# hridaybavle/semantic_slam

Hardware: AMD Instinct MI355X
Metric: graph-optimize LM iters/sec (5k poses, 1k landmarks) (higher is better)
Workload: dtype f64

## Files before the change

semantic_slam_amd/csrc/chol_plan.hpp:

```cpp
#pragma once
#include <algorithm>
#include <array>
#include <cstdint>
#include <cstdio>
#include <cstdlib>
#include <cstring>
#include <functional>
#include <map>
#include <queue>
#include <string>
#include <unordered_map>
#include <utility>
#include <vector>

namespace sslam {
#ifdef SSLAM_PLAN_TIMERS
#include <chrono>
#define SSLAM_PT_INIT auto pt_ = std::chrono::steady_clock::now();
#define SSLAM_PT(name) { auto n_ = std::chrono::steady_clock::now(); fprintf(stderr, "[plan-timer] %-14s %.3f ms\n", name, std::chrono::duration<double, std::milli>(n_ - pt_).count()); pt_ = n_; }
#else
#define SSLAM_PT_INIT
#define SSLAM_PT(name)
#endif

struct ColMeta { int xoff, yoff, dim, graph, b0, nb, nbi, base, f0, f1, piece, ilevel; };

struct BlkMeta { int off, src, xoff_row, yoff_row, coldiag, colyoff, info, as0; };
constexpr int kBlkFmt = 1 << 8, kBlkDiag = 1 << 9, kBlkRowIn = 1 << 10, kBlkNasShift = 16;
inline int blk_irank_bits(int r) { return ((r & 31) << 11) | ((r >> 5) << 24); }
#if defined(__HIPCC__)
__host__ __device__
#endif
inline int blk_irank(int info) { return ((info >> 11) & 31) | (((info >> 24) & 255) << 5); }

struct AsmSrc { int uoff, uyoff; };
struct FwdMeta { int off, yoff; };

struct UpdMeta { unsigned ab, xk; };
constexpr unsigned kUpdDi6 = 1u << 28;
constexpr unsigned kUpdDk6 = 1u << 29;
constexpr unsigned kUpdDiag = 1u << 30;
constexpr unsigned kUpdDj6 = 1u << 31;
constexpr int kUpdLocalMax = 1 << 16, kUpdYMax = 1 << 13, kUpdRightYMax = 1 << 12;
#if defined(__HIPCC__)
#define SSLAM_HD_INLINE __host__ __device__ inline
#else
#define SSLAM_HD_INLINE inline
#endif
SSLAM_HD_INLINE int upd_ua(const UpdMeta& r) { return (int)(r.ab & 0xFFFFu); }
SSLAM_HD_INLINE int upd_ub(const UpdMeta& r) { return (int)(r.ab >> 16); }
SSLAM_HD_INLINE int upd_yk(const UpdMeta& r) { return (int)(r.xk & 0x1FFFu); }
SSLAM_HD_INLINE int upd_rt(const UpdMeta& r) { return (int)(r.xk & 0xFFFFu); }
SSLAM_HD_INLINE int upd_ry(const UpdMeta& r) { return (int)((r.xk >> 16) & 0xFFFu); }
inline UpdMeta upd_make(int ua_local, int ub_local, int yk_local, unsigned flags) { return UpdMeta{(unsigned)ua_local | ((unsigned)ub_local << 16), (unsigned)yk_local | flags}; }
inline UpdMeta upd_make_right(int ua_local, int ub_local, int tl, int yl, unsigned flags) { return UpdMeta{(unsigned)ua_local | ((unsigned)ub_local << 16), (unsigned)tl | ((unsigned)yl << 16) | flags}; }

}
#include "front_plan.hpp"
namespace sslam {

struct ItemMeta { int u0, n, tloff, flags; };
constexpr int kItemSole = 1;
constexpr int kItemSlotShift = 1, kItemSlotMask = 0x7FF, kItemYShift = 12;
struct MbMeta { int tloff, ps0, n, info; };
struct RCol { int u0, n; };
struct ILevel { int c0, c1, b0, b1, it0, it1, mb0, mb1; };

struct UItem { int u0, n, uoff, flags, s0, ns, uyoff, pad; };
constexpr int kUItemDi6 = 1 << 12, kUItemDj6 = 1 << 13, kUItemDiag = 1 << 14;
struct UMb { int uoff, ps0, n, info, s0, ns, uyoff, pad; };

struct PieceMeta { int graph, c0, nc, b0, nb, lbase, lsize, y0, ysize, ilv0, nilv, iit0, nit_i, iu0, nu_i, imb0, nimb, as0, nas, uit0, nuit, umb0, numb,
                   uu0, nuu, us0, nus, n36, n18, nint, pad3, pad4, nu4, nu2, nu1, pad5; };

inline int blk_doubles(int di, int dj) { return (di * dj + 1) & ~1; }
constexpr int kItemDoubles = 42;
constexpr int kMaxILevels = 64;

struct SymGraph { int prow0, nprow, lrow0, nlrow; int pp0 = 0, pp1 = 0, pl0 = 0, pl1 = 0, ll0 = 0, ll1 = 0; };
struct SymIn {
  int B = 0, nPr = 0, nLr = 0;
  std::vector<SymGraph> seg;
  std::vector<std::pair<int, int>> ppoff, plblk;
  std::vector<std::pair<int, int>> llblk;
  int64_t hll_base = 0, hpp_off_base = 0, hpl_base = 0, hll_off_base = 0;
};
// ... 34 lines not shown
        for (const char* v : legacy)
          if (getenv(v)) fprintf(stderr, "[sslam] %s is no longer read: plan options go through SSLAM_CHOL_OPTS=\"key=value,...\" (chol_plan.hpp CholOpts)\n", v);
      }
    }
    const char* e = getenv("SSLAM_CHOL_OPTS");
    if (!e) return;
    std::string str(e);
    size_t pos = 0;
    while (pos < str.size()) {
      size_t end = str.find(',', pos);
      if (end == std::string::npos) end = str.size();
      const std::string kv = str.substr(pos, end - pos);
      pos = end + 1;
      const size_t eq = kv.find('=');
      if (eq == std::string::npos) continue;
      const std::string k = kv.substr(0, eq), v = kv.substr(eq + 1);
      const int iv = atoi(v.c_str());
      if (k == "cap_leaf") cap_leaf = iv; else if (k == "cap_mid") cap_mid = iv; else if (k == "cap_tail") cap_tail = iv;
      else if (k == "max_blocks") max_blocks = iv; else if (k == "tail_width") tail_width = iv; else if (k == "mid_width") mid_width = iv;
      else if (k == "nt_leaf") { nt_leaf = iv; nt_leaf_set = true; } else if (k == "nt_mid") nt_mid = iv; else if (k == "nt_ftail") nt_ftail = iv; else if (k == "nt_bleaf") nt_bleaf = iv; else if (k == "nt_bmid") nt_bmid = iv; else if (k == "nt_btail") nt_btail = iv; else if (k == "nt_tail") nt_tail = iv;
      else if (k == "min_chunk") min_chunk = std::max(1, iv); else if (k == "split_min") split_min = std::max(2, iv);
      else if (k == "pcap_leaf") pcap_leaf = iv; else if (k == "pcap_mid") pcap_mid = iv; else if (k == "pcap_tail") pcap_tail = iv;
      else if (k == "group_cap") group_cap = iv; else if (k == "group_blocks") group_blocks = iv; else if (k == "ustage") ustage = iv;
      else if (k == "order_bits_max") order_bits_max = iv; else if (k == "flow") flow = iv; else if (k == "front") front = iv; else if (k == "compact") compact = iv; else if (k == "dump") dump = iv != 0;
      else if (k == "order") order = (v == "mindeg" || v == "0") ? 0 : 1;
      else if (k == "order_mul") order_mul = atof(v.c_str()); else if (k == "order_add") order_add = iv;
      else fprintf(stderr, "[sslam] SSLAM_CHOL_OPTS: unknown key '%s'\n", k.c_str());
    }
  }
  bool nt_leaf_set = false;
};

inline bool chol_throughput_regime(int B, int block_rows) { return B >= 32 || (B >= 2 && block_rows >= 8000); }
inline bool chol_opts_normalise(CholOpts& opt, int B, int block_rows) {
  auto one_of = [](int v, std::initializer_list<int> set) { return std::find(set.begin(), set.end(), v) != set.end(); };
  if (opt.nt_tail != 1024) opt.nt_tail = 512;
  if (!one_of(opt.nt_leaf, {-1, 128, 256, 512, 1024})) opt.nt_leaf = 64;
  if (!one_of(opt.nt_mid, {256, 512})) opt.nt_mid = 128;
  if (opt.nt_tail == 1024) opt.nt_ftail = 1024;
  else if (!one_of(opt.nt_ftail, {128, 256, 1024})) opt.nt_ftail = 512;
  if (!one_of(opt.nt_btail, {128, 256})) opt.nt_btail = 512;
  for (int* nt : {&opt.nt_bleaf, &opt.nt_bmid})
    if (*nt <= 0) *nt = 0;
    else if (!one_of(*nt, {128, 256, 512, 1024})) *nt = 64;
  const bool want_flow = opt.flow != 0 && B < 8 && !chol_throughput_regime(B, block_rows) && opt.nt_tail == 512 && opt.group_cap <= 0 && !opt.nt_leaf_set;
  if (want_flow) { opt.nt_leaf = opt.nt_tail; opt.mid_width = 0; }
  return want_flow;
}

struct CholHost {
  int ncol = 0, nlevels = 0, dim = 0, B = 0, npiece = 0;
  int64_t lnz = 0;
  int64_t unz = 0;
  std::vector<ColMeta> col; std::vector<BlkMeta> blk; std::vector<UpdMeta> upd; std::vector<ItemMeta> item; std::vector<MbMeta> mb;
  std::vector<ILevel> ilv; std::vector<PieceMeta> piece;
  std::vector<AsmSrc> asrc, usrc; std::vector<FwdMeta> fwd; std::vector<UItem> uitem; std::vector<UMb> umb;
  std::vector<RCol> rcol; std::vector<UpdMeta> rupd;
  std::vector<int> lvl_ptr, lvl_cols;
  std::vector<int> plv_ptr, plv_pieces;
  std::vector<PieceMeta> lpiece;
  std::vector<int> tail_ptr, tail_pieces;
  std::vector<int> plv_lds_f, plv_lds_b;
  std::vector<int> plv_nt, plv_cls;
  int tail_lds_f = 0, tail_lds_b = 0;
  int nt_leaf = 64, nt_mid = 128, nt_tail = 512, nt_ftail = 256, nt_bleaf = 0, nt_bmid = 0, nt_btail = 0, ustage = 0;
  bool front = false;
  std::string front_why;
  std::vector<uint32_t> fblob;
  std::vector<FrontGrp> fgrp, lfgrp;
  std::vector<int> plv_lds_ff;
  int tail_lds_ff = 0;
  int64_t funz = 0;
  std::string error;
};

namespace chol_detail {

struct GraphSym {
  std::vector<int> order;
  std::vector<int> cs_start, cs_len, cs_idx;
};

inline void min_degree(int n, std::vector<std::vector<int>>& adj, GraphSym& out) {
  std::vector<char> done(n, 0);
  using Item = std::pair<int, int>;
  std::priority_queue<Item, std::vector<Item>, std::greater<Item>> pq;
  for (int v = 0; v < n; ++v) { std::sort(adj[v].begin(), adj[v].end()); pq.push({(int)adj[v].size(), v}); }
  out.order.clear(); out.order.reserve(n);
  out.cs_start.assign(n, 0); out.cs_len.assign(n, 0); out.cs_idx.clear();
  std::vector<int> merged;
  while (!pq.empty()) {
    const Item it = pq.top(); pq.pop();
    const int v = it.second;
    if (done[v] || it.first != (int)adj[v].size()) continue;
    done[v] = 1;
    out.order.push_back(v);
    std::vector<int>& nb = adj[v];
    out.cs_start[v] = (int)out.cs_idx.size(); out.cs_len[v] = (int)nb.size(); out.cs_idx.insert(out.cs_idx.end(), nb.begin(), nb.end());
    for (int u : nb) {
      std::vector<int>& au = adj[u];
      merged.clear();
      merged.reserve(au.size() + nb.size());
      std::set_union(au.begin(), au.end(), nb.begin(), nb.end(), std::back_inserter(merged));
      au.clear();
      for (int w : merged) if (w != u && w != v) au.push_back(w);
      pq.push({(int)au.size(), u});
    }
// ... 436 lines not shown
    }
  }
  std::vector<int> plev(npiece, 0);
  for (int j = 0; j < ncol; ++j)
    if (bp[j + 1] - bp[j] > 1) {
      const int pp = col_piece[brow[bp[j] + 1]], pj = col_piece[j];
      if (pp != pj) plev[pp] = std::max(plev[pp], plev[pj] + 1);
    }
  int nplv = 0;
  for (int p = 0; p < npiece; ++p) if (!piece_tail[p]) nplv = std::max(nplv, plev[p] + 1);
  out.plv_ptr.assign(nplv + 1, 0);
  for (int p = 0; p < npiece; ++p) if (!piece_tail[p]) out.plv_ptr[plev[p] + 1]++;
  for (int l = 0; l < nplv; ++l) out.plv_ptr[l + 1] += out.plv_ptr[l];
  out.plv_pieces.resize(out.plv_ptr[nplv]);
  {
    std::vector<int> cursor(out.plv_ptr.begin(), out.plv_ptr.end() - 1);
    for (int p = 0; p < npiece; ++p) if (!piece_tail[p]) out.plv_pieces[cursor[plev[p]]++] = p;
  }
  out.tail_ptr.assign(B + 1, 0);
  for (int p = 0; p < npiece; ++p) if (piece_tail[p]) out.tail_ptr[out.piece[p].graph + 1]++;
  for (int g = 0; g < B; ++g) out.tail_ptr[g + 1] += out.tail_ptr[g];
  out.tail_pieces.resize(out.tail_ptr[B]);
  {
    std::vector<int> cursor(out.tail_ptr.begin(), out.tail_ptr.end() - 1);
    for (int p = 0; p < npiece; ++p) if (piece_tail[p]) out.tail_pieces[cursor[out.piece[p].graph]++] = p;
  }
  out.col.assign(ncol, ColMeta{});
  out.blk.assign(nblk, BlkMeta{});
  std::vector<int> block_col(nblk), col_nbi(ncol, 0);
  {
    std::vector<int> rowcnt(ncol + 1, 0);
    for (int j = 0; j < ncol; ++j) for (int t = bp[j] + 1; t < bp[j + 1]; ++t) rowcnt[brow[t] + 1]++;
    for (int j = 0; j < ncol; ++j) rowcnt[j + 1] += rowcnt[j];
    out.fwd.resize(rowcnt[ncol]);
    std::vector<int> cursor(rowcnt.begin(), rowcnt.end() - 1);
    for (int j = 0; j < ncol; ++j) {
      const int pj = col_piece[j];
      int nbi = 0;
      for (int t = bp[j]; t < bp[j + 1]; ++t) if (col_piece[brow[t]] == pj) ++nbi;
      for (int t = bp[j]; t < bp[j] + nbi; ++t) if (col_piece[brow[t]] != pj) { out.error = "in-piece rows of a column are not a prefix"; return -1; }
      col_nbi[j] = nbi;
      out.col[j] = ColMeta{col_xoff[j], col_yoff[j], col_dim[j], col_graph[j], bp[j], bp[j + 1] - bp[j], nbi, boff[bp[j]], rowcnt[j], rowcnt[j + 1], pj, col_il[j]};
      for (int t = bp[j]; t < bp[j + 1]; ++t) {
        const int i = brow[t];
        block_col[t] = j;
        BlkMeta& bm = out.blk[t];
        bm.off = boff[t]; bm.src = bsrc[t];
        bm.xoff_row = col_xoff[i]; bm.yoff_row = col_yoff[i]; bm.coldiag = boff[bp[j]]; bm.colyoff = col_yoff[j]; bm.as0 = 0;
        bm.info = col_dim[i] | (col_dim[j] << 4) | (bfmt[t] ? kBlkFmt : 0) | (t == bp[j] ? kBlkDiag : 0) | (col_piece[i] == pj ? kBlkRowIn : 0);
        if (t > bp[j]) out.fwd[cursor[i]++] = FwdMeta{boff[t] | (col_dim[j] == 6 ? (int)0x80000000u : 0), col_yoff[j]};
      }
    }
  }
  for (int p = 0; p < npiece; ++p) {
    PieceMeta& pm = out.piece[p];
    int r = 0;
    for (int t = pm.b0; t < pm.b0 + pm.nb; ++t)
      if (out.blk[t].info & kBlkRowIn) {
        if (r >= 8192) { out.error = "piece with more than 8191 row-in-piece blocks"; return -1; }
        out.blk[t].info |= blk_irank_bits(r++);
      }
    pm.nint = r;
  }
  SSLAM_PT("levels+cols")
  struct URec { int a, b, uoff, uy, comp; };
  std::vector<std::vector<URec>> inbox(npiece);
  std::vector<std::vector<int>> comp_R(ncomp);
  out.upd.clear(); out.item.clear(); out.mb.clear(); out.ilv.clear(); out.asrc.clear(); out.usrc.clear(); out.uitem.clear(); out.umb.clear();
  out.rupd.clear(); out.rcol.assign(ncol, RCol{0, 0});
  bool right_ok = true;
  std::vector<int> piece_pmax(npiece, 0);
  int64_t ucur = 0;
  struct UB { int comp, a, b; };
  struct OwnRec { int blk, ua, ubo, k; };
  struct SrcRec { int blk; AsmSrc s; };
  struct IU { int t, ua, ub2, k; };
  struct AsmRec { int t; AsmSrc s; };
  std::vector<UB> ub;
  std::vector<int> comps, ctab_base, ctab, rix, iu_ptr, as_ptr, own_ptr, src_ptr, cur1, cur2, cur3, cur4, bi0, bi1, order, uoffs;
  std::vector<OwnRec> own_flat, own_s;
  std::vector<SrcRec> src_flat;
  std::vector<IU> iu_flat, iu_s;
  std::vector<AsmRec> asm_flat;
  std::vector<AsmSrc> as_s, src_s;
  std::vector<int> lens, comp_uy;
  std::vector<UItem> uit_s;
  auto fit_chunk = [&](int lo, int hi, int pcap) {
    auto nonsole = [&](int chunk) { int s2 = 0; for (int n : lens) { const int k = (n + chunk - 1) / chunk; if (k > 1) s2 += k; } return s2; };
    if (lo >= hi || nonsole(lo) <= pcap) return lo;
    int a = lo, b = hi;
    while (b - a > 1) { const int m = a + (b - a) / 2; if (nonsole(m) <= pcap) b = m; else a = m; }
    return b;
  };
  for (int p = 0; p < npiece; ++p) {
    PieceMeta& pm = out.piece[p];
    const int nt = piece_tail[p] ? opt.nt_tail : (piece_cls[p] == 1 ? opt.nt_mid : opt.nt_leaf);
    const int slots = nt / 4;
    const int pcap = piece_tail[p] ? opt.pcap_tail : (piece_cls[p] == 1 ? opt.pcap_mid : opt.pcap_leaf);
    comps.clear();
    for (int j = pm.c0; j < pm.c0 + pm.nc; ++j) {
      if (comps.empty() || std::find(comps.begin(), comps.end(), col_comp[j]) == comps.end()) comps.push_back(col_comp[j]);
      std::vector<int>& R = comp_R[col_comp[j]];
      for (int t = bp[j] + col_nbi[j]; t < bp[j + 1]; ++t) R.push_back(brow[t]);
    }
    std::sort(comps.begin(), comps.end());
    for (int c : comps) {
      std::vector<int>& R = comp_R[c];
      std::sort(R.begin(), R.end());
      R.erase(std::unique(R.begin(), R.end()), R.end());
    }
    ub.clear();
    ctab_base.assign(comps.size() + 1, 0);
    for (size_t ci = 0; ci < comps.size(); ++ci) { const int r = (int)comp_R[comps[ci]].size(); ctab_base[ci + 1] = ctab_base[ci] + r * (r + 1) / 2; }
    ctab.assign(ctab_base.back(), -1);
    auto ublock = [&](int comp, int a, int b2) -> int {
// ... 180 lines not shown
        if (diag) {
          const std::vector<int>& R = comp_R[x.comp];
          uy = comp_uy[std::lower_bound(comps.begin(), comps.end(), x.comp) - comps.begin()] + 6 * (int)(std::lower_bound(R.begin(), R.end(), x.a) - R.begin());
        }
        const unsigned tpk = (di == 6 ? kUpdDi6 : 0u) | (diag ? kUpdDiag : 0u) | (dj == 6 ? kUpdDj6 : 0u);
        const int u0 = (int)out.upd.size() - pm.uu0;
        for (int w = own_ptr[q]; w < own_ptr[q + 1]; ++w) { const OwnRec& u = own_s[w]; out.upd.push_back(upd_make(u.ua - pm.lbase, u.ubo - pm.lbase, col_yoff[u.k] - pm.y0, tpk | (col_dim[u.k] == 6 ? kUpdDk6 : 0u))); }
        const int n = own_ptr[q + 1] - own_ptr[q];
        const int s0 = (int)out.usrc.size() - pm.us0;
        for (int w = src_ptr[q]; w < src_ptr[q + 1]; ++w) out.usrc.push_back(src_s[w]);
        const int ns = src_ptr[q + 1] - src_ptr[q];
        const int k = std::max(1, (n + chunk - 1) / chunk);
        const int shape = (di == 6 ? kUItemDi6 : 0) | (dj == 6 ? kUItemDj6 : 0) | (diag ? kUItemDiag : 0);
        for (int qq = 0; qq < k; ++qq) {
          const int a2 = u0 + qq * chunk, b2 = std::min(u0 + n, a2 + chunk);
          out.uitem.push_back(UItem{a2, std::max(0, b2 - a2), uoffs[q], shape | (k == 1 ? kItemSole : ((ps + qq) << kItemSlotShift)), s0, ns, uy, 0});
        }
        if (k > 1) { out.umb.push_back(UMb{uoffs[q], ps, k, di | (dj << 4) | (diag ? kBlkDiag : 0), s0, ns, uy, 0}); ps += k; }
        if (comp_dest[x.comp] < 0) { out.error = "a root component has an update matrix"; return -1; }
        inbox[comp_dest[x.comp]].push_back(URec{x.a, x.b, uoffs[q], uy, x.comp});
      }
      piece_pmax[p] = std::max(piece_pmax[p], ps);
      ucur = cur;
      {
        auto cls = [](const UItem& im) {
          if (!(im.flags & kItemSole)) return 3;
          const int t = ((im.flags & kUItemDi6) ? 2 : 1) * ((im.flags & kUItemDj6) ? 2 : 1);
          return t == 4 ? 0 : (t == 2 ? 1 : 2);
        };
        int cnt[4] = {0, 0, 0, 0};
        for (size_t i = item_first; i < out.uitem.size(); ++i) cnt[cls(out.uitem[i])]++;
        pm.nu4 = cnt[0]; pm.nu2 = cnt[1]; pm.nu1 = cnt[2];
        int at[4] = {0, cnt[0], cnt[0] + cnt[1], cnt[0] + cnt[1] + cnt[2]};
        uit_s.assign(out.uitem.begin() + item_first, out.uitem.end());
        for (const UItem& im : uit_s) out.uitem[item_first + at[cls(im)]++] = im;
      }
    }
    pm.nuit = (int)out.uitem.size() - pm.uit0;
    pm.numb = (int)out.umb.size() - pm.umb0;
    pm.nuu = (int)out.upd.size() - pm.uu0;
    pm.nus = (int)out.usrc.size() - pm.us0;
  }
  out.unz = ucur;
  SSLAM_PT("piece loop")
  if (!right_ok) { out.rupd.clear(); out.rcol.assign(ncol, RCol{0, 0}); }
  auto lds_f = [&](int p) {
    const PieceMeta& pm = out.piece[p];
    const int ustage = (piece_cls[p] >= 1 || !opt.ustage) ? 0 : 4 * pm.nuit + 4 * pm.numb + ((pm.nuu + 1) & ~1) + pm.nus + 2;
    return 4 * pm.nilv + ((pm.lsize + 1) & ~1) + 2 * ((pm.ysize + 1) & ~1) + 4 * pm.nb + 3 * pm.nc + 2 * pm.nit_i + ((pm.nu_i + 1) & ~1) + 2 * pm.nimb + pm.nas + ustage +
           kItemDoubles * piece_pmax[p] + 8 + (piece_cls[p] >= 1 ? pm.nc + 2 : 0);
  };
  auto lds_b = [&](int p) {
    const PieceMeta& pm = out.piece[p];
    return 4 * pm.nilv + 36 * pm.nint + ((pm.ysize + 1) & ~1) + 7 * pm.nb + 3 * pm.nc + 12;
  };
  {
    std::vector<int> ptr{0}, launch_order, lnt, lcls;
    launch_order.reserve(out.plv_pieces.size());
    const int cut[3] = {640, 853, 1280};
    for (int l = 0; l < nplv; ++l) {
      std::vector<int> ps, pmid;
      for (int q = out.plv_ptr[l]; q < out.plv_ptr[l + 1]; ++q) (piece_cls[out.plv_pieces[q]] == 1 ? pmid : ps).push_back(out.plv_pieces[q]);
      const int n = (int)ps.size();
      if (n >= opt.split_min) {
        std::stable_sort(ps.begin(), ps.end(), [&](int a, int b) { return lds_b(a) < lds_b(b); });
        int q0 = 0;
        for (int k = 0; k < 3 && q0 < n; ++k) {
          int q1 = q0;
          while (q1 < n && lds_b(ps[q1]) <= cut[k]) ++q1;
          if (q1 - q0 >= opt.split_min / 2 && n - q1 >= opt.split_min / 2) { for (int q = q0; q < q1; ++q) launch_order.push_back(ps[q]); ptr.push_back((int)launch_order.size()); lnt.push_back(opt.nt_leaf); lcls.push_back(0); q0 = q1; }
        }
        for (int q = q0; q < n; ++q) launch_order.push_back(ps[q]);
      } else {
        for (int p : ps) launch_order.push_back(p);
      }
      if ((int)launch_order.size() > ptr.back()) { ptr.push_back((int)launch_order.size()); lnt.push_back(opt.nt_leaf); lcls.push_back(0); }
      if (!pmid.empty()) { for (int p : pmid) launch_order.push_back(p); ptr.push_back((int)launch_order.size()); lnt.push_back(opt.nt_mid); lcls.push_back(1); }
    }
    out.plv_nt = lnt; out.plv_cls = lcls;
    out.plv_pieces = launch_order;
    out.plv_ptr = ptr;
  }
  const int nlaunch = (int)out.plv_ptr.size() - 1;
  out.lpiece.clear();
  out.lpiece.reserve(npiece);
  for (int p : out.plv_pieces) out.lpiece.push_back(out.piece[p]);
  for (int p : out.tail_pieces) out.lpiece.push_back(out.piece[p]);
  out.plv_lds_f.assign(nlaunch, 0); out.plv_lds_b.assign(nlaunch, 0);
  for (int l = 0; l < nlaunch; ++l)
    for (int q = out.plv_ptr[l]; q < out.plv_ptr[l + 1]; ++q) {
      out.plv_lds_f[l] = std::max(out.plv_lds_f[l], lds_f(out.plv_pieces[q]));
      out.plv_lds_b[l] = std::max(out.plv_lds_b[l], lds_b(out.plv_pieces[q]));
    }
  for (int p : out.tail_pieces) { out.tail_lds_f = std::max(out.tail_lds_f, lds_f(p)); out.tail_lds_b = std::max(out.tail_lds_b, lds_b(p)); }
  if (opt.front > 0) {
    FrontHost F;
    front_build(FrontIn{ncol, npiece, ncomp, bp, brow, boff, bsrc, bfmt, col_comp, col_piece, col_dim, col_xoff, col_yoff, col_il, comp_parent, comp_R}, out.piece, out.ilv, F);
    for (int p = 0; p < npiece && F.ok; ++p) {
      const int nt = piece_tail[p] ? opt.nt_ftail : (piece_cls[p] == 1 ? opt.nt_mid : opt.nt_leaf);
      for (int l = 0; l < out.piece[p].nilv; ++l) {
        const ILevel& lv = out.ilv[out.piece[p].ilv0 + l];
        if (lv.c1 - lv.c0 > 2 * (nt / 8)) { F.ok = false; F.why = "a level of a piece has more columns than the workgroup's teams hold"; break; }
      }
    }
    out.front = F.ok; out.front_why = F.why;
    if (F.ok) {
      out.fblob.swap(F.blob); out.fgrp.swap(F.grp); out.funz = F.unz;
      out.lfgrp.reserve(npiece);
      for (int p : out.plv_pieces) out.lfgrp.push_back(out.fgrp[p]);
      for (int p : out.tail_pieces) out.lfgrp.push_back(out.fgrp[p]);
      out.plv_lds_ff.assign(nlaunch, 0);
      for (int l = 0; l < nlaunch; ++l)
// ... 22 lines not shown
```

semantic_slam_amd/csrc/sslam_chol.hip:

```cpp
#include <hip/hip_runtime.h>
#include <algorithm>
#include <cstdio>
#include <cstring>
#include <mutex>
#include <type_traits>
#include <vector>

#include "../../include/sslam.h"
#include "graph_engine.hpp"
#include "chol_plan.hpp"

namespace sslam {

struct CholView {
  int ncol, nlevels, dim, npiece;
  const ColMeta* col;
  const BlkMeta* blk;
  const UpdMeta* upd;
  const ItemMeta* item;
  const MbMeta* mb;
  const ILevel* ilv;
  const PieceMeta* piece;
  const PieceMeta* lpiece;
  int ltail0;
  const AsmSrc* asrc;
  const AsmSrc* usrc;
  const UItem* uitem;
  const UMb* umb;
  const RCol* rcol;
  const UpdMeta* rupd;
  const int* plv_pieces;
  const int* tail_ptr;
  const int* tail_pieces;
  double* Lval;
  double* Uval;
  double* y;
  int* fail;
  const unsigned* fblob;
  const FrontGrp* lfgrp;
  int flat_L;
  long long* dbg;
};

struct SpecLanes {
  int K = 0;
  LmState* lm = nullptr;
  double *Lval = nullptr, *Uval = nullptr, *y = nullptr, *x = nullptr, *pose_trial = nullptr, *lmk_trial = nullptr, *part_e = nullptr, *part_a = nullptr;
  int *fail = nullptr, *flow = nullptr;
  int* err = nullptr;
  const double *pose_cur = nullptr, *lmk_cur = nullptr;
  long long sL = 0, sU = 0, sy = 0, sx = 0, spose = 0, slmk = 0, spe = 0, spa = 0, sflow = 0;
  int g0 = 0, g1 = 0;
  int after = 0;
  int* ctl = nullptr;
};

struct CholPlan {
  CholView C{};
  SpecLanes spec{};
  std::vector<int> plv_ptr, plv_lds_f, plv_lds_b, plv_nt, plv_cls;
  std::vector<int> plv_lds_ff;
  int tail_lds_ff = 0;
  bool front = false;
  int tail_lds_f = 0, tail_lds_b = 0, tail_total = 0, nt_tail = 512, nt_ftail = 256, nt_bleaf = 0, nt_bmid = 0, nt_btail = 0, ustage = 0;
  std::vector<void*> allocs;
  DevArena* arena = nullptr;
  int64_t lnz = 0, unz = 0;
  std::vector<int> lp_graph;
  std::vector<int> c_ptr;
  int* d_idx = nullptr;
// ... 658 lines not shown
  SSLAM_STAMP(6)
  if (C.flat_L) {
    D2* dst = reinterpret_cast<D2*>(C.Lval + pm.lbase);
    const D2* src = reinterpret_cast<const D2*>(smL);
    for (int e = tid; e < (pm.lsize >> 1); e += NT) dst[e] = src[e];
  } else {
    double* dst = C.Lval + pm.lbase;
    const int nA = pm.n36, nB = pm.n18, nC = pm.nb - nA - nB, eA = 36 * nA, eB = eA + 18 * nB;
    const float rA = 1.0f / (float)max(nA, 1), rB = 1.0f / (float)max(nB, 1), rC = 1.0f / (float)max(nC, 1);
    for (int t = tid; t < eA; t += NT) { const int k = (int)(((float)t + 0.5f) * rA), i = t - k * nA; dst[t] = smL[i * 36 + k]; }
    for (int t = tid; t < 18 * nB; t += NT) { const int k = (int)(((float)t + 0.5f) * rB), i = t - k * nB; dst[eA + t] = smL[eA + i * 18 + k]; }
    for (int t = tid; t < 9 * nC; t += NT) { const int k = (int)(((float)t + 0.5f) * rC), i = t - k * nC; dst[eB + t] = smL[eB + i * 10 + k]; }
  }
  for (int e = tid; e < pm.ysize; e += NT) C.y[pm.y0 + e] = smY[e];
  SSLAM_STAMP(7)
  if (dbg && threadIdx.x == 0) { dbg[8] += 1; dbg[9] += pm.nilv; dbg[10] += pm.nuit; dbg[11] += pm.nit_i; }
}
#undef SSLAM_STAMP

template <int NT, bool USTAGE, bool RIGHT = false>
__global__ __launch_bounds__(NT, 4) void k_chol_pieces(BatchView V, CholView C, int begin, const int* __restrict__ idx) {
  extern __shared__ double sm[];
  const PieceMeta pm = C.lpiece[idx ? idx[blockIdx.x] : begin + blockIdx.x];
  if (!V.lm[pm.graph].in_trial) return;
  chol_piece<NT, USTAGE, RIGHT>(V, C, pm, sm, (C.dbg && blockIdx.x == 0) ? C.dbg + 16 : nullptr);
}

template <int NT>
__global__ __launch_bounds__(NT) void k_chol_tail(BatchView V, CholView C, const int* __restrict__ idx) {
  extern __shared__ double sm[];
  const int g = idx ? idx[blockIdx.x] : blockIdx.x;
  if (!V.lm[g].in_trial) return;
  const int q1 = C.tail_ptr[g + 1];
  for (int q = C.tail_ptr[g]; q < q1; ++q) {
    if (C.rupd) chol_piece<NT, false, true>(V, C, C.lpiece[C.ltail0 + q], sm, (C.dbg && g == 0) ? C.dbg : nullptr);
    else chol_piece<NT, false, false>(V, C, C.lpiece[C.ltail0 + q], sm, (C.dbg && g == 0) ? C.dbg : nullptr);
    __threadfence_block();
    __syncthreads();
  }
}

#define SSLAM_BSTAMP(k)                                                         \
  if (dbg) {                                                                    \
    const long long now_ = clock64();                                           \
    if (threadIdx.x == 0) dbg[k] += now_ - tprev;                               \
    tprev = now_;                                                               \
  }
template <int NT>
__device__ __forceinline__ void chol_piece_backward(const CholView& C, const PieceMeta pm, const double* __restrict__ y, double* x, double* sm, long long* dbg) {
  ILevel* s_lvb = reinterpret_cast<ILevel*>(sm);
  long long tprev = dbg ? clock64() : 0;
  const int tid = threadIdx.x;
  const int Yp = (pm.ysize + 1) & ~1;
  double* smI = sm + 4 * pm.nilv;
  double* smX = smI + 36 * pm.nint;
  double* smE = smX + Yp;
  int2* sBlk = reinterpret_cast<int2*>(smE + 6 * pm.nb);
  int4* sCol = reinterpret_cast<int4*>(sBlk + pm.nb + (pm.nb & 1));
  int* sXoff = reinterpret_cast<int*>(sCol + pm.nc);
  const int nA = pm.n36, nB = pm.n18, nC = pm.nb - nA - nB, eA = 36 * nA, eB = eA + 18 * nB;
  const double y_r = y[pm.y0 + min(tid, pm.ysize - 1)];
  const ILevel lv_r = C.ilv[pm.ilv0 + min(tid, max(pm.nilv - 1, 0))];
  const ColMeta col_r = C.col[pm.c0 + min(tid, pm.nc - 1)];
  for (int b = tid; b < pm.nb; b += NT) {
    const BlkMeta bm = C.blk[pm.b0 + b];
    const int di = bm.info & 15, dj = (bm.info >> 4) & 15;
    const bool in = bm.info & kBlkRowIn;
    const int ol = bm.off - pm.lbase;
    int st, n, i;
    if (ol < eA) { st = 0; n = nA; i = ol / 36; }
    else if (ol < eB) { st = eA; n = nB; i = (ol - eA) / 18; }
    else { st = eB; n = nC; i = (ol - eB) / 10; }
    const double* __restrict__ g = C.Lval + pm.lbase + st + i;
    if (in) {
      const int lo = 36 * blk_irank(bm.info);
      sBlk[b] = make_int2(lo | (di << 24) | (dj << 28), bm.yoff_row - pm.y0);
      double* o = smI + lo;
      if (dj == 6) {
        for (int r = 0; r < di; r += 3) {
          double v[18];
#pragma unroll
          for (int k = 0; k < 18; ++k) v[k] = g[(size_t)(r * 6 + k) * n];
#pragma unroll
          for (int k = 0; k < 18; ++k) o[r * 6 + k] = v[k];
        }
      } else {
        for (int r = 0; r < di; r += 3) {
          double v[9];
#pragma unroll
          for (int k = 0; k < 9; ++k) v[k] = g[(size_t)(r * 3 + k) * n];
#pragma unroll
          for (int k = 0; k < 9; ++k) o[r * 3 + k] = v[k];
        }
      }
    } else {
      const double* xi = x + bm.xoff_row;
      double sv[6] = {0, 0, 0, 0, 0, 0};
      if (dj == 6) {
        for (int r = 0; r < di; r += 3) {
          double v[18];
          const double x0 = xi[r], x1 = xi[r + 1], x2 = xi[r + 2];
#pragma unroll
          for (int k = 0; k < 18; ++k) v[k] = g[(size_t)(r * 6 + k) * n];
#pragma unroll
          for (int c = 0; c < 6; ++c) { sv[c] += v[c] * x0; sv[c] += v[6 + c] * x1; sv[c] += v[12 + c] * x2; }
        }
      } else {
        for (int r = 0; r < di; r += 3) {
          double v[9];
          const double x0 = xi[r], x1 = xi[r + 1], x2 = xi[r + 2];
#pragma unroll
          for (int k = 0; k < 9; ++k) v[k] = g[(size_t)(r * 3 + k) * n];
#pragma unroll
          for (int c = 0; c < 3; ++c) { sv[c] += v[c] * x0; sv[c] += v[3 + c] * x1; sv[c] += v[6 + c] * x2; }
        }
      }
#pragma unroll
      for (int c = 0; c < 6; ++c) smE[b * 6 + c] = sv[c];
    }
  }
  if (tid < pm.ysize) smX[tid] = y_r;
  for (int e = tid + NT; e < pm.ysize; e += NT) smX[e] = y[pm.y0 + e];
  if (tid < pm.nilv) s_lvb[tid] = lv_r;
  for (int i = tid + NT; i < pm.nilv; i += NT) s_lvb[i] = C.ilv[pm.ilv0 + i];
  if (tid < pm.nc) { sCol[tid] = make_int4(col_r.b0 - pm.b0, col_r.dim | (col_r.nb << 8) | (col_r.nbi << 20), col_r.yoff - pm.y0, 0); sXoff[tid] = col_r.xoff; }
  for (int c = tid + NT; c < pm.nc; c += NT) {
    const ColMeta cm = C.col[pm.c0 + c];
    sCol[c] = make_int4(cm.b0 - pm.b0, cm.dim | (cm.nb << 8) | (cm.nbi << 20), cm.yoff - pm.y0, 0);
    sXoff[c] = cm.xoff;
  }
  __syncthreads();
  SSLAM_BSTAMP(0)
  for (int t = tid; t < pm.nc * 8; t += NT) {
    const int cidx = t >> 3, c = t & 7;
    const int4 cm = sCol[cidx];
    const int dj = cm.y & 255, nb = (cm.y >> 8) & 0xFFF, nbi = cm.y >> 20;
    if (c >= dj) continue;
    double acc = 0;
    for (int bi = nbi; bi < nb; ++bi) acc += smE[(cm.x + bi) * 6 + c];
    smX[cm.z + c] -= acc;
  }
  __syncthreads();
  SSLAM_BSTAMP(1)
  for (int il = pm.nilv - 1; il >= 0; --il) {
    const ILevel lv = s_lvb[il];
    const int ncols = lv.c1 - lv.c0;
    int Q = 1;
    while (Q < 8 && ncols * 16 * Q <= NT) Q *= 2;
    const int team = tid / (8 * Q), lt = tid % (8 * Q), nteams = NT / (8 * Q);
    const int c = lt & 7, q = lt >> 3;
    for (int ci = team; ci < ncols; ci += nteams) {
      const int4 cm = sCol[lv.c0 - pm.c0 + ci];
      const int dj = cm.y & 255, nbi = cm.y >> 20;
      const int cc = min(c, dj - 1);
      const double* D = smI + (sBlk[cm.x].x & 0xFFFFFF);
      double acc = 0;
      for (int bi = 1 + q; bi < nbi; bi += Q) {
        const int2 bm = sBlk[cm.x + bi];
        const double* Bk = smI + (bm.x & 0xFFFFFF) + cc;
        const double* xi = smX + bm.y;
        double s = Bk[0] * xi[0] + Bk[dj] * xi[1] + Bk[2 * dj] * xi[2];
        if (((bm.x >> 24) & 15) == 6) s += Bk[3 * dj] * xi[3] + Bk[4 * dj] * xi[4] + Bk[5 * dj] * xi[5];
        acc += s;
      }
      if (Q > 1) acc += __shfl_xor(acc, 8, 64);
      if (Q > 2) acc += __shfl_xor(acc, 16, 64);
      if (Q > 4) acc += __shfl_xor(acc, 32, 64);
      if (q == 0 && c < dj) smX[cm.z + c] -= acc;
      __builtin_amdgcn_fence(__ATOMIC_ACQ_REL, "wavefront");
      __builtin_amdgcn_wave_barrier();
      double tv[6], xv[6];
#pragma unroll
      for (int r = 0; r < 6; ++r) tv[r] = smX[cm.z + min(r, dj - 1)];
      if (dj == 6) {
#pragma unroll
        for (int r = 5; r >= 0; --r) {
          double a = tv[r];
#pragma unroll
          for (int s2 = 5; s2 > r; --s2) a -= D[s2 * 6 + r] * xv[s2];
          xv[r] = a / D[r * 6 + r];
        }
      } else {
#pragma unroll
        for (int r = 2; r >= 0; --r) {
          double a = tv[r];
#pragma unroll
          for (int s2 = 2; s2 > r; --s2) a -= D[s2 * 3 + r] * xv[s2];
          xv[r] = a / D[r * 3 + r];
        }
        xv[3] = xv[4] = xv[5] = 0.0;
      }
      __builtin_amdgcn_wave_barrier();
      if (q == 0 && c < dj) smX[cm.z + c] = c == 0 ? xv[0] : c == 1 ? xv[1] : c == 2 ? xv[2] : c == 3 ? xv[3] : c == 4 ? xv[4] : xv[5];
    }
    __syncthreads();
  }
  SSLAM_BSTAMP(2)
  for (int cidx = tid; cidx < pm.nc; cidx += NT) {
    const int4 cm = sCol[cidx];
    const int dj = cm.y & 255;
    double* xo = x + sXoff[cidx];
#pragma unroll
    for (int c = 0; c < 6; ++c) if (c < dj) xo[c] = smX[cm.z + c];
  }
  SSLAM_BSTAMP(3)
  if (dbg && threadIdx.x == 0) { dbg[4] += 1; dbg[5] += pm.nilv; dbg[6] += pm.nb; }
}
#undef SSLAM_BSTAMP

template <int NT>
__global__ __launch_bounds__(NT, NT == 64 ? 8 : 1) void k_chol_back_pieces(CholView C, int begin, const double* __restrict__ y, double* x, const LmState* __restrict__ lm, const int* __restrict__ idx) {
  extern __shared__ double sm[];
  const PieceMeta pm = C.lpiece[idx ? idx[blockIdx.x] : begin + blockIdx.x];
  if (lm && !lm[pm.graph].in_trial) return;
  chol_piece_backward<NT>(C, pm, y, x, sm, (C.dbg && blockIdx.x == 0) ? C.dbg + 40 : nullptr);
}
template <int NT>
__global__ __launch_bounds__(NT) void k_chol_back_tail(CholView C, const double* __restrict__ y, double* x, const LmState* __restrict__ lm, const int* __restrict__ idx) {
  extern __shared__ double sm[];
  const int g = idx ? idx[blockIdx.x] : blockIdx.x;
  if (lm && !lm[g].in_trial) return;
  const int q0 = C.tail_ptr[g];
  for (int q = C.tail_ptr[g + 1] - 1; q >= q0; --q) {
    chol_piece_backward<NT>(C, C.lpiece[C.ltail0 + q], y, x, sm, (C.dbg && g == 0) ? C.dbg + 32 : nullptr);
    __threadfence_block();
    __syncthreads();
  }
}

__device__ __forceinline__ void marginal_path_forward(const CholView& C, const int* __restrict__ cols, int P, int D, double* Y, double* sD,
                                                      int4* prec, int* pyoff) {
  const int lane = threadIdx.x;
  const double* __restrict__ L = C.Lval;
  for (int t = lane; t < P; t += 64) {
    const ColMeta cm = C.col[cols[t]];
    prec[t] = make_int4(cm.b0, cm.nb, cm.base, cm.dim);
    pyoff[t] = cm.yoff;
  }
  for (int e = lane; e < P * 36; e += 64) Y[e] = 0.0;
  __syncthreads();
  if (lane < D) Y[lane * 6 + lane] = 1.0;
// ... 620 lines not shown
  if (!h.empty()) SSLAM_HIP_TRY(hipMemcpyAsync(p, h.data(), h.size() * sizeof(T), hipMemcpyHostToDevice, s));
  *out = (const T*)p;
  return 0;
}
}

void chol_sym_input(const Batch& b, SymIn& in) {
  in.B = b.V.B; in.nPr = b.V.nPr; in.nLr = b.V.nLr;
  in.seg.resize(b.seg.size());
  for (size_t g = 0; g < b.seg.size(); ++g) in.seg[g] = SymGraph{b.seg[g].prow0, b.seg[g].nprow, b.seg[g].lrow0, b.seg[g].nlrow};
  in.ppoff = b.ppoff; in.plblk = b.plblk; in.llblk = b.llblk;
  in.hll_base = b.hll_base; in.hpp_off_base = b.hpp_off_base; in.hpl_base = b.hpl_base; in.hll_off_base = b.hll_off_base;
}

int chol_spec_mode(const Batch& b) {
  static const int env = [] { const char* e = getenv("SSLAM_LM_SPEC"); return e ? std::max(0, std::min(2, atoi(e))) : -1; }();
  return env >= 0 ? env : b.graphs[0]->opt.speculative;
}
int chol_plan_build(Batch& b) {
  struct HostTimer { Batch& b; std::chrono::steady_clock::time_point t0 = std::chrono::steady_clock::now();
                     ~HostTimer() { b.plan_build_ms += std::chrono::duration<double, std::milli>(std::chrono::steady_clock::now() - t0).count(); } } host_timer{b};
  if (b.chol) { chol_plan_free(b.chol); b.chol = nullptr; }
  SSLAM_HIP_TRY(hipSetDevice(b.device));
  SymIn in;
  chol_sym_input(b, in);
  CholOpts opt;
  opt.from_env();
  const int flow_mode = opt.flow;
  const bool want_flow = chol_opts_normalise(opt, b.V.B, b.V.nPr + b.V.nLr);
  CholHost H;
  if (chol_symbolic(in, opt, H)) return set_error(SSLAM_ERR_NUMERIC, "Cholesky plan: %s", H.error.c_str());
  CholPlan* P = new CholPlan();
  b.chol = P;
  P->arena = b.arena;
  P->allow_compact = opt.compact != 0;
  CholView& C = P->C;
  C.ncol = H.ncol; C.nlevels = H.nlevels; C.dim = H.dim; C.npiece = H.npiece;
  P->plv_ptr = H.plv_ptr; P->plv_lds_f = H.plv_lds_f; P->plv_lds_b = H.plv_lds_b; P->plv_nt = H.plv_nt; P->plv_cls = H.plv_cls;
  P->tail_lds_f = H.tail_lds_f; P->tail_lds_b = H.tail_lds_b; P->tail_total = (int)H.tail_pieces.size(); P->nt_tail = H.nt_tail; P->nt_ftail = H.nt_ftail; P->nt_bleaf = H.nt_bleaf; P->nt_bmid = H.nt_bmid; P->nt_btail = H.nt_btail; P->ustage = H.ustage;
  P->lnz = H.lnz;
  {
    std::vector<int> yoff_col(H.dim + 1, -1);
    for (int j = 0; j < H.ncol; ++j) yoff_col[H.col[j].yoff] = j;
    P->h_cparent.assign(H.ncol, -1);
    P->h_xoff_col.assign(H.dim + 1, -1);
    for (int j = 0; j < H.ncol; ++j) {
      if (H.col[j].nb > 1) P->h_cparent[j] = yoff_col[H.blk[H.col[j].b0 + 1].yoff_row];
      P->h_xoff_col[H.col[j].xoff] = j;
    }
  }
  int rc;
  if ((rc = up_to_dev(*P, b.stream, H.col, &C.col))) return rc;
  if ((rc = up_to_dev(*P, b.stream, H.blk, &C.blk))) return rc;
  if ((rc = up_to_dev(*P, b.stream, H.upd, &C.upd))) return rc;
  if ((rc = up_to_dev(*P, b.stream, H.item, &C.item))) return rc;
  if ((rc = up_to_dev(*P, b.stream, H.mb, &C.mb))) return rc;
  if ((rc = up_to_dev(*P, b.stream, H.ilv, &C.ilv))) return rc;
  if ((rc = up_to_dev(*P, b.stream, H.piece, &C.piece))) return rc;
  if ((rc = up_to_dev(*P, b.stream, H.lpiece, &C.lpiece))) return rc;
  C.ltail0 = (int)H.plv_pieces.size();
  P->lp_graph.resize(H.lpiece.size());
  for (size_t q = 0; q < H.lpiece.size(); ++q) P->lp_graph[q] = H.lpiece[q].graph;
  std::vector<int2> dep;
  if (want_flow) {
    const int np = (int)H.lpiece.size();
    std::vector<int> lidx(H.npiece, -1);
    int q = 0;
    for (int p : H.plv_pieces) lidx[p] = q++;
    for (int p : H.tail_pieces) lidx[p] = q++;
    dep.assign(np, make_int2(-1, 0));
    bool ok = q == np;
    for (int i = 0; i < np && ok; ++i) {
      const int par = H.lpiece[i].pad4;
      if (par == -2) ok = false;
      else if (par >= 0) { const int j = lidx[par]; if (j <= i) ok = false; else { dep[i].x = j; dep[j].y++; } }
    }
    P->flow = ok;
  }
  if ((rc = up_to_dev(*P, b.stream, H.asrc, &C.asrc))) return rc;
  if ((rc = up_to_dev(*P, b.stream, H.usrc, &C.usrc))) return rc;
  if ((rc = up_to_dev(*P, b.stream, H.uitem, &C.uitem))) return rc;
  if ((rc = up_to_dev(*P, b.stream, H.umb, &C.umb))) return rc;
  {
    C.rcol = nullptr; C.rupd = nullptr;
    if (!H.rupd.empty()) {
      if ((rc = up_to_dev(*P, b.stream, H.rcol, &C.rcol))) return rc;
      if ((rc = up_to_dev(*P, b.stream, H.rupd, &C.rupd))) return rc;
    }
  }
  if ((rc = up_to_dev(*P, b.stream, H.plv_pieces, &C.plv_pieces))) return rc;
  if ((rc = up_to_dev(*P, b.stream, H.tail_ptr, &C.tail_ptr))) return rc;
  if ((rc = up_to_dev(*P, b.stream, H.tail_pieces, &C.tail_pieces))) return rc;
  C.fblob = nullptr; C.lfgrp = nullptr;
  if (H.front) {
    if ((rc = up_to_dev(*P, b.stream, H.fblob, (const uint32_t**)&C.fblob))) return rc;
    if ((rc = up_to_dev(*P, b.stream, H.lfgrp, &C.lfgrp))) return rc;
    P->front = true; P->plv_lds_ff = H.plv_lds_ff; P->tail_lds_ff = H.tail_lds_ff;
  } else if (opt.front != 0 && chol_throughput_regime(b.V.B, b.V.nPr + b.V.nLr)) {
    fprintf(stderr, "[sslam] Cholesky plan without front tables (%s): the record kernels run\n", H.front_why.c_str());
  }
  void* p = nullptr;
  auto plan_alloc = [&](void** q, size_t bytes) -> int {
    if (P->arena) {
      *q = P->arena->take(bytes, true);
      if (*q) P->arena->note_direct(*q, bytes);
      return *q ? 0 : set_error(SSLAM_ERR_HIP, "device allocation of %zu bytes failed", bytes);
// ... 584 lines not shown
```

semantic_slam_amd/csrc/sslam_graph.hip:

```cpp
#include <hip/hip_runtime.h>
#include <rccl/rccl.h>
#include <dlfcn.h>
#include <algorithm>
#include <chrono>
#include <cmath>
#include <cstdio>
#include <cstring>
#include <functional>
#include <map>
#include <memory>
#include <string>
#include <unordered_map>
#include <thread>
#include <vector>

#include "../../include/sslam.h"
#include "graph_host.hpp"
#include "graph_kernels.hpp"
#include "sslam_common.hpp"
#include "graph_engine.hpp"
#include "chol_plan.hpp"

namespace sslam {

// ... 2799 lines not shown
  h->b.profiling = enable != 0;
  h->b.timers.clear();
  return 0;
}
int sslam_batch_kernel_time(sslam_batch* h, const char* name, double* total_ms, int64_t* launches) {
  if (!h || !name) return set_error(SSLAM_ERR_INVALID, "null argument");
  if (!h->parts.empty()) {
    double t = 0; int64_t n = 0;
    for (sslam_batch* p : h->parts) { double a = 0; int64_t c = 0; sslam_batch_kernel_time(p, name, &a, &c); t += a; n += c; }
    if (total_ms) *total_ms = t;
    if (launches) *launches = n;
    return 0;
  }
  auto it = h->b.timers.find(name);
  if (total_ms) *total_ms = it == h->b.timers.end() ? 0.0 : it->second.total_ms;
  if (launches) *launches = it == h->b.timers.end() ? 0 : it->second.launches;
  return 0;
}

struct sslam_debug_plan { CholHost H; int64_t h_total = 0; std::vector<int> ppoff, plblk; int sc[16] = {0}; };
void* sslam_debug_plan_create(sslam_graph* const* graphs, int n) {
  if (!graphs || n <= 0) { set_error(SSLAM_ERR_INVALID, "empty batch"); return nullptr; }
  Batch b;
  for (int i = 0; i < n; ++i) { if (!graphs[i]) { set_error(SSLAM_ERR_INVALID, "null graph"); return nullptr; } b.graphs.push_back(&graphs[i]->g); }
  static const bool timing = getenv("SSLAM_TIMING") != nullptr;
  const auto t0 = std::chrono::steady_clock::now();
  if (batch_build(b, true) != 0) return nullptr;
  const auto t1 = std::chrono::steady_clock::now();
  SymIn in;
  chol_sym_input(b, in);
  CholOpts opt;
  opt.from_env();
  chol_opts_normalise(opt, b.V.B, b.V.nPr + b.V.nLr);
  sslam_debug_plan* P = new sslam_debug_plan();
  P->h_total = b.V.h_total;
  for (auto& q : b.ppoff) { P->ppoff.push_back(q.first); P->ppoff.push_back(q.second); }
  for (auto& q : b.plblk) { P->plblk.push_back(q.first); P->plblk.push_back(q.second); }
  P->sc[11] = b.V.nPr; P->sc[12] = b.V.nLr; P->sc[13] = (int)b.hll_base; P->sc[14] = (int)b.hpp_off_base; P->sc[15] = (int)b.hpl_base;
  if (chol_symbolic(in, opt, P->H)) { set_error(SSLAM_ERR_NUMERIC, "Cholesky plan: %s", P->H.error.c_str()); delete P; return nullptr; }
  if (timing) fprintf(stderr, "[timing] host plan: batch tables %.3f ms, symbolic Cholesky %.3f ms\n", std::chrono::duration<double, std::milli>(t1 - t0).count(),
                      std::chrono::duration<double, std::milli>(std::chrono::steady_clock::now() - t1).count());
  return P;
}
void sslam_debug_plan_destroy(void* p) { delete (sslam_debug_plan*)p; }
int64_t sslam_debug_plan_array(void* p, const char* name, void* out, int64_t cap_bytes) {
  if (!p || !name) return set_error(SSLAM_ERR_INVALID, "null argument");
  const CholHost& H = ((sslam_debug_plan*)p)->H;
  const std::string k(name);
  const void* src = nullptr; int64_t bytes = 0;
  const sslam_debug_plan& DP = *(sslam_debug_plan*)p;
  int scal[17] = {H.ncol, H.nlevels, H.dim, H.B, H.npiece, (int)H.lnz, H.tail_lds_f, H.tail_lds_b, H.nt_leaf, H.nt_tail, (int)DP.h_total,
                  DP.sc[11], DP.sc[12], DP.sc[13], DP.sc[14], DP.sc[15], (int)H.unz};
#define ARR(nm, vec) if (k == nm) { src = (vec).data(); bytes = (int64_t)(vec).size() * sizeof((vec)[0]); }
  ARR("col", H.col) ARR("blk", H.blk) ARR("upd", H.upd) ARR("item", H.item) ARR("mb", H.mb) ARR("ilv", H.ilv) ARR("piece", H.piece)
  ARR("lvl_ptr", H.lvl_ptr) ARR("lvl_cols", H.lvl_cols) ARR("plv_ptr", H.plv_ptr) ARR("plv_pieces", H.plv_pieces)
  ARR("ppoff", DP.ppoff) ARR("plblk", DP.plblk) ARR("tail_ptr", H.tail_ptr)
  ARR("asrc", H.asrc) ARR("usrc", H.usrc) ARR("fwd", H.fwd) ARR("uitem", H.uitem) ARR("umb", H.umb) ARR("tail_pieces", H.tail_pieces) ARR("plv_lds_f", H.plv_lds_f) ARR("plv_lds_b", H.plv_lds_b)
  ARR("rcol", H.rcol) ARR("rupd", H.rupd) ARR("plv_nt", H.plv_nt) ARR("plv_cls", H.plv_cls)
  ARR("fblob", H.fblob) ARR("fgrp", H.fgrp) ARR("plv_lds_ff", H.plv_lds_ff)
#undef ARR
  int fscal[4] = {H.front ? 1 : 0, (int)H.funz, H.tail_lds_ff, 0};
  if (k == "fscalars") { src = fscal; bytes = sizeof fscal; }
  if (k == "scalars") { src = scal; bytes = sizeof scal; }
  static const char* known[] = {"col", "blk", "upd", "item", "mb", "ilv", "piece", "lvl_ptr", "lvl_cols", "plv_ptr", "plv_pieces", "ppoff", "plblk",
                                "tail_ptr", "tail_pieces", "plv_lds_f", "plv_lds_b", "scalars", "asrc", "usrc", "fwd", "uitem", "umb", "rcol", "rupd", "plv_nt", "plv_cls",
                                "fblob", "fgrp", "plv_lds_ff", "fscalars"};
  bool ok = false;
  for (const char* q : known) ok |= (k == q);
  if (!ok) return set_error(SSLAM_ERR_INVALID, "unknown plan array '%s'", name);
  if (out && cap_bytes >= bytes && bytes > 0) memcpy(out, src, (size_t)bytes);
  return bytes;
}

}
```

Baseline: 34850.

## Pack backward-solve shared-memory block storage with per-block offsets and triangular diagonals

The backward triangular-solve kernel now lays out per-piece LDS block storage compactly. A host-computed per-block offset array (blo) replaces fixed 36-double slots per in-piece block and a 6-double slot per out-of-piece block. Diagonal blocks are stored as packed lower triangles, and out-of-piece partial sums are placed at variable 3- or 6-wide offsets. The goal is a smaller LDS footprint per piece so more pieces fit or occupancy rises, and the piece-class LDS cut thresholds are lowered to match. The cost is an extra global metadata array and more complex indexing.

```diff
diff --git a/semantic_slam_amd/csrc/chol_plan.hpp b/semantic_slam_amd/csrc/chol_plan.hpp
--- a/semantic_slam_amd/csrc/chol_plan.hpp
+++ b/semantic_slam_amd/csrc/chol_plan.hpp
@@ -32,6 +32,10 @@
 __host__ __device__
 #endif
 inline int blk_irank(int info) { return ((info >> 11) & 31) | (((info >> 24) & 255) << 5); }
+inline int blk_back_doubles(int info) {
+  const int di = info & 15, dj = (info >> 4) & 15;
+  return !(info & (1 << 10)) ? dj : ((info & (1 << 9)) ? dj * (dj + 1) / 2 : di * dj);
+}
 
 struct AsmSrc { int uoff, uyoff; };
 struct FwdMeta { int off, yoff; };
@@ -172,7 +176,7 @@
   int ncol = 0, nlevels = 0, dim = 0, B = 0, npiece = 0;
   int64_t lnz = 0;
   int64_t unz = 0;
-  std::vector<ColMeta> col; std::vector<BlkMeta> blk; std::vector<UpdMeta> upd; std::vector<ItemMeta> item; std::vector<MbMeta> mb;
+  std::vector<ColMeta> col; std::vector<BlkMeta> blk; std::vector<int> blo; std::vector<UpdMeta> upd; std::vector<ItemMeta> item; std::vector<MbMeta> mb;
   std::vector<ILevel> ilv; std::vector<PieceMeta> piece;
   std::vector<AsmSrc> asrc, usrc; std::vector<FwdMeta> fwd; std::vector<UItem> uitem; std::vector<UMb> umb;
   std::vector<RCol> rcol; std::vector<UpdMeta> rupd;
@@ -715,15 +719,21 @@
       }
     }
   }
+  out.blo.assign(nblk, 0);
+  std::vector<int> piece_back(npiece, 0);
   for (int p = 0; p < npiece; ++p) {
     PieceMeta& pm = out.piece[p];
-    int r = 0;
+    int r = 0, at = 0;
     for (int t = pm.b0; t < pm.b0 + pm.nb; ++t)
       if (out.blk[t].info & kBlkRowIn) {
         if (r >= 8192) { out.error = "piece with more than 8191 row-in-piece blocks"; return -1; }
         out.blk[t].info |= blk_irank_bits(r++);
+        out.blo[t] = at; at += blk_back_doubles(out.blk[t].info);
       }
     pm.nint = r;
+    for (int t = pm.b0; t < pm.b0 + pm.nb; ++t)
+      if (!(out.blk[t].info & kBlkRowIn)) { out.blo[t] = at; at += blk_back_doubles(out.blk[t].info); }
+    piece_back[p] = at;
   }
   SSLAM_PT("levels+cols")
   struct URec { int a, b, uoff, uy, comp; };
@@ -1010,12 +1020,12 @@
   };
   auto lds_b = [&](int p) {
     const PieceMeta& pm = out.piece[p];
-    return 4 * pm.nilv + 36 * pm.nint + ((pm.ysize + 1) & ~1) + 7 * pm.nb + 3 * pm.nc + 12;
+    return 4 * pm.nilv + ((pm.ysize + 1) & ~1) + ((pm.nb + 1) & ~1) + 2 * pm.nc + ((pm.nc + 1) >> 1) + piece_back[p];
   };
   {
     std::vector<int> ptr{0}, launch_order, lnt, lcls;
     launch_order.reserve(out.plv_pieces.size());
-    const int cut[3] = {640, 853, 1280};
+    const int cut[3] = {500, 666, 1000};
     for (int l = 0; l < nplv; ++l) {
       std::vector<int> ps, pmid;
       for (int q = out.plv_ptr[l]; q < out.plv_ptr[l + 1]; ++q) (piece_cls[out.plv_pieces[q]] == 1 ? pmid : ps).push_back(out.plv_pieces[q]);
diff --git a/semantic_slam_amd/csrc/sslam_chol.hip b/semantic_slam_amd/csrc/sslam_chol.hip
--- a/semantic_slam_amd/csrc/sslam_chol.hip
+++ b/semantic_slam_amd/csrc/sslam_chol.hip
@@ -16,6 +16,7 @@
   int ncol, nlevels, dim, npiece;
   const ColMeta* col;
   const BlkMeta* blk;
+  const int* blo;
   const UpdMeta* upd;
   const ItemMeta* item;
   const MbMeta* mb;
@@ -780,18 +781,18 @@
   long long tprev = dbg ? clock64() : 0;
   const int tid = threadIdx.x;
   const int Yp = (pm.ysize + 1) & ~1;
-  double* smI = sm + 4 * pm.nilv;
-  double* smX = smI + 36 * pm.nint;
-  double* smE = smX + Yp;
-  int2* sBlk = reinterpret_cast<int2*>(smE + 6 * pm.nb);
+  double* smX = sm + 4 * pm.nilv;
+  int2* sBlk = reinterpret_cast<int2*>(smX + Yp);
   int4* sCol = reinterpret_cast<int4*>(sBlk + pm.nb + (pm.nb & 1));
   int* sXoff = reinterpret_cast<int*>(sCol + pm.nc);
+  double* smI = reinterpret_cast<double*>(sXoff + pm.nc + (pm.nc & 1));
   const int nA = pm.n36, nB = pm.n18, nC = pm.nb - nA - nB, eA = 36 * nA, eB = eA + 18 * nB;
   const double y_r = y[pm.y0 + min(tid, pm.ysize - 1)];
   const ILevel lv_r = C.ilv[pm.ilv0 + min(tid, max(pm.nilv - 1, 0))];
   const ColMeta col_r = C.col[pm.c0 + min(tid, pm.nc - 1)];
   for (int b = tid; b < pm.nb; b += NT) {
     const BlkMeta bm = C.blk[pm.b0 + b];
+    const int lo = C.blo[pm.b0 + b];
     const int di = bm.info & 15, dj = (bm.info >> 4) & 15;
     const bool in = bm.info & kBlkRowIn;
     const int ol = bm.off - pm.lbase;
@@ -800,10 +801,27 @@
     else if (ol < eB) { st = eA; n = nB; i = (ol - eA) / 18; }
     else { st = eB; n = nC; i = (ol - eB) / 10; }
     const double* __restrict__ g = C.Lval + pm.lbase + st + i;
-    if (in) {
-      const int lo = 36 * blk_irank(bm.info);
+    double* o = smI + lo;
+    if (bm.info & kBlkDiag) {
       sBlk[b] = make_int2(lo | (di << 24) | (dj << 28), bm.yoff_row - pm.y0);
-      double* o = smI + lo;
+      if (dj == 6) {
+#pragma unroll
+        for (int r = 0; r < 6; r += 3) {
+          double v[18];
+#pragma unroll
+          for (int k = 0; k < 18; ++k) v[k] = g[(size_t)(r * 6 + k) * n];
+#pragma unroll
+          for (int k = 0; k < 18; ++k) if (k % 6 <= r + k / 6) o[(r + k / 6) * (r + k / 6 + 1) / 2 + k % 6] = v[k];
+        }
+      } else {
+        double v[9];
+#pragma unroll
+        for (int k = 0; k < 9; ++k) v[k] = g[(size_t)k * n];
+#pragma unroll
+        for (int k = 0; k < 9; ++k) if (k % 3 <= k / 3) o[(k / 3) * (k / 3 + 1) / 2 + k % 3] = v[k];
+      }
+    } else if (in) {
+      sBlk[b] = make_int2(lo | (di << 24) | (dj << 28), bm.yoff_row - pm.y0);
       if (dj == 6) {
         for (int r = 0; r < di; r += 3) {
           double v[18];
@@ -843,8 +861,9 @@
           for (int c = 0; c < 3; ++c) { sv[c] += v[c] * x0; sv[c] += v[3 + c] * x1; sv[c] += v[6 + c] * x2; }
         }
       }
-#pragma unroll
-      for (int c = 0; c < 6; ++c) smE[b * 6 + c] = sv[c];
+      sBlk[b] = make_int2(lo, 0);
+      o[0] = sv[0]; o[1] = sv[1]; o[2] = sv[2];
+      if (dj == 6) { o[3] = sv[3]; o[4] = sv[4]; o[5] = sv[5]; }
     }
   }
   if (tid < pm.ysize) smX[tid] = y_r;
@@ -864,8 +883,10 @@
     const int4 cm = sCol[cidx];
     const int dj = cm.y & 255, nb = (cm.y >> 8) & 0xFFF, nbi = cm.y >> 20;
     if (c >= dj) continue;
+    if (nbi >= nb) continue;
+    const double* e = smI + sBlk[cm.x + nbi].x + c;
     double acc = 0;
-    for (int bi = nbi; bi < nb; ++bi) acc += smE[(cm.x + bi) * 6 + c];
+    for (int bi = nbi; bi < nb; ++bi) acc += e[(bi - nbi) * dj];
     smX[cm.z + c] -= acc;
   }
   __syncthreads();
@@ -905,16 +926,16 @@
         for (int r = 5; r >= 0; --r) {
           double a = tv[r];
 #pragma unroll
-          for (int s2 = 5; s2 > r; --s2) a -= D[s2 * 6 + r] * xv[s2];
-          xv[r] = a / D[r * 6 + r];
+          for (int s2 = 5; s2 > r; --s2) a -= D[s2 * (s2 + 1) / 2 + r] * xv[s2];
+          xv[r] = a / D[r * (r + 1) / 2 + r];
         }
       } else {
 #pragma unroll
         for (int r = 2; r >= 0; --r) {
           double a = tv[r];
 #pragma unroll
-          for (int s2 = 2; s2 > r; --s2) a -= D[s2 * 3 + r] * xv[s2];
-          xv[r] = a / D[r * 3 + r];
+          for (int s2 = 2; s2 > r; --s2) a -= D[s2 * (s2 + 1) / 2 + r] * xv[s2];
+          xv[r] = a / D[r * (r + 1) / 2 + r];
         }
         xv[3] = xv[4] = xv[5] = 0.0;
       }
@@ -1641,6 +1662,7 @@
   int rc;
   if ((rc = up_to_dev(*P, b.stream, H.col, &C.col))) return rc;
   if ((rc = up_to_dev(*P, b.stream, H.blk, &C.blk))) return rc;
+  if ((rc = up_to_dev(*P, b.stream, H.blo, &C.blo))) return rc;
   if ((rc = up_to_dev(*P, b.stream, H.upd, &C.upd))) return rc;
   if ((rc = up_to_dev(*P, b.stream, H.item, &C.item))) return rc;
   if ((rc = up_to_dev(*P, b.stream, H.mb, &C.mb))) return rc;
diff --git a/semantic_slam_amd/csrc/sslam_graph.hip b/semantic_slam_amd/csrc/sslam_graph.hip
--- a/semantic_slam_amd/csrc/sslam_graph.hip
+++ b/semantic_slam_amd/csrc/sslam_graph.hip
@@ -2875,7 +2875,7 @@
   int scal[17] = {H.ncol, H.nlevels, H.dim, H.B, H.npiece, (int)H.lnz, H.tail_lds_f, H.tail_lds_b, H.nt_leaf, H.nt_tail, (int)DP.h_total,
                   DP.sc[11], DP.sc[12], DP.sc[13], DP.sc[14], DP.sc[15], (int)H.unz};
 #define ARR(nm, vec) if (k == nm) { src = (vec).data(); bytes = (int64_t)(vec).size() * sizeof((vec)[0]); }
-  ARR("col", H.col) ARR("blk", H.blk) ARR("upd", H.upd) ARR("item", H.item) ARR("mb", H.mb) ARR("ilv", H.ilv) ARR("piece", H.piece)
+  ARR("col", H.col) ARR("blk", H.blk) ARR("blo", H.blo) ARR("upd", H.upd) ARR("item", H.item) ARR("mb", H.mb) ARR("ilv", H.ilv) ARR("piece", H.piece)
   ARR("lvl_ptr", H.lvl_ptr) ARR("lvl_cols", H.lvl_cols) ARR("plv_ptr", H.plv_ptr) ARR("plv_pieces", H.plv_pieces)
   ARR("ppoff", DP.ppoff) ARR("plblk", DP.plblk) ARR("tail_ptr", H.tail_ptr)
   ARR("asrc", H.asrc) ARR("usrc", H.usrc) ARR("fwd", H.fwd) ARR("uitem", H.uitem) ARR("umb", H.umb) ARR("tail_pieces", H.tail_pieces) ARR("plv_lds_f", H.plv_lds_f) ARR("plv_lds_b", H.plv_lds_b)
@@ -2887,7 +2887,7 @@
   if (k == "scalars") { src = scal; bytes = sizeof scal; }
   static const char* known[] = {"col", "blk", "upd", "item", "mb", "ilv", "piece", "lvl_ptr", "lvl_cols", "plv_ptr", "plv_pieces", "ppoff", "plblk",
                                 "tail_ptr", "tail_pieces", "plv_lds_f", "plv_lds_b", "scalars", "asrc", "usrc", "fwd", "uitem", "umb", "rcol", "rupd", "plv_nt", "plv_cls",
-                                "fblob", "fgrp", "plv_lds_ff", "fscalars"};
+                                "fblob", "fgrp", "plv_lds_ff", "fscalars", "blo"};
   bool ok = false;
   for (const char* q : known) ok |= (k == q);
   if (!ok) return set_error(SSLAM_ERR_INVALID, "unknown plan array '%s'", name);
```

Result: no change. 35280 (median of 3 runs) (+1.2%).
